# DecodeGenetics/graphtyper

Hardware: AMD Instinct MI355X
Metric: aligned+genotyped reads/sec over 1 Mb graph region; VCF bit-identical (higher is better)
Workload: dtype u64/u32 integer (2-bit k-mer keys, byte compares, u32 atomics)

## Files before the change

graphtyper_amd/csrc/gtx_api.hip:

```cpp
#include <hip/hip_runtime.h>
#include <chrono>

#include <algorithm>
#include <cstdio>
#include <cstdlib>
#include <cstring>
#include <memory>
#include <string>

#include "gtx_ctx.hpp"

#include <map>
#include "gtx_devmem.hpp"
#include "wave_hip.hpp"
#include "align_core.hpp"
#include "gtx_hbm_passes.hpp"
#include "score_core.hpp"
#include "score_replay.hpp"

namespace gtx
{
#ifdef GTX_PROF
constexpr uint64_t PROF_LOG_ENTRIES = 1u << 16, PROF_LOG_ENTRY = 16;
#else
// ... 1885 lines not shown
  CallScratch * const s = a.s;
  AlignRequest const & r = a.r;
  uint32_t const n = r.n_reads;
  uint32_t * const counters = s->d_counters;
  char const * fb = std::getenv("GTX_FORCE_SECOND_PASS");
  uint32_t const force = fb ? static_cast<uint32_t>(std::atoi(fb)) : 0u;
  uint32_t const n_cu = static_cast<uint32_t>(c->n_cu > 0 ? c->n_cu : 256);
  uint32_t const force_both = static_cast<uint32_t>(c->params.force_align_both_orientations != 0);
  char const * e4 = std::getenv("GTX_EXPRESS4");
  char const * eh = std::getenv("GTX_HINT");
  bool const four = !(e4 && e4[0] == '0');
  a.hinted = four && !(eh && eh[0] == '0');
  bool const wide = e4 && e4[0] == 'w' ? true : e4 && e4[0] == 'l' ? false : c->express4_wide;
  uint64_t const chunks = (static_cast<uint64_t>(n) + TASK_CHUNK - 1) / TASK_CHUNK;
  uint32_t const express4_per_cu = static_cast<uint32_t>(wide ? c->express4_wide_blocks_per_cu : c->express4_blocks_per_cu);
  a.mark(0, r.stream);
  if (a.hinted)
  {
    bool const sv_skips_express = c->params.is_sv_graph != 0 && force == 0;
    char const * hb = std::getenv("GTX_HINT_BUILD");
    bool const hint_dense = hb && hb[0] == 'd' ? true : hb && hb[0] == 'l' ? false : c->express4_wide;
    bool const hint_long = r.seq_stride > HintGeom<AlignCfg::KC>::ROW_BYTES;
    uint32_t const hint_threads = 64u * ((hint_long || hint_dense) ? GTX_HINT_WAVES : GTX_HINT_WAVES_LEAN);
    hipLaunchKernelGGL(hint_long ? gtx_align_hinted_long_kernel : hint_dense ? gtx_align_hinted_dense_kernel : gtx_align_hinted_kernel,
                       dim3((n + hint_threads - 1u) / hint_threads), dim3(hint_threads), 0, r.stream, c->dev_graph, c->dev_index, r.seq, r.seq_stride,
                       r.meta, n, r.records, r.rec_words, force_both, s->d_queue1.get(), s->d_queue.get(), reinterpret_cast<unsigned long long *>(counters + 2),
                       static_cast<uint32_t>(force != 0 || (eh && eh[0] == 'd')) | (sv_skips_express ? 4u : 0u)
#ifdef GTX_PROF
                         | (eh && eh[0] == 'x' ? 2u : 0u)
#endif
                         ,
                       r.task_flags, r.compact, a.timed && s->h_span.get() ? s->d_span : static_cast<unsigned long long *>(nullptr), a.var_masks);
    if (!hip_ok(hipGetLastError(), "gtx_align_hinted_kernel launch"))
      return GTX_ERR_HIP;
  }
  a.mark(1, r.stream);
  if (r.front_event)
  {
    (void)hipEventRecord(r.front_event, r.stream);
    if (r.tail_stream && r.tail_stream != r.stream)
    {
      (void)hipStreamWaitEvent(r.tail_stream, r.front_event, 0);
      a.sq = r.tail_stream;
    }
  }
  if (a.hinted)
  {
    uint32_t const blocks4q = static_cast<uint32_t>(std::min<uint64_t>((static_cast<uint64_t>(n) + 3u) / 4u, static_cast<uint64_t>(n_cu) * express4_per_cu));
// ... 1093 lines not shown
```

graphtyper_amd/csrc/gtx_flat.hpp:

```cpp
#pragma once
#include <algorithm>
#include <cstdlib>
#include <cstdint>
#include <string>
#include <vector>

#include "../../include/gtx.h"

namespace gtx
{
constexpr uint32_t K = GTX_K;
constexpr uint32_t INVALID = GTX_INVALID_ID;
constexpr uint32_t SPECIAL_START = GTX_SPECIAL_START;
constexpr uint32_t POS_BUCKET_SHIFT = 6;
constexpr uint32_t MAX_ALLELES = 32u * GTX_WIDE_MASK_WORDS;

struct alignas(8) uint2_t
{
  uint32_t x, y;
};

struct alignas(16) DevLabel
{
  uint32_t start, end;
// ... 55 lines not shown
};

constexpr uint32_t HINT_WIN_BEFORE = 160, HINT_WIN_ALLELE_MAX = 64, HINT_WIN_STRIDE = 384;
struct HintWindow
{
  uint32_t site, allele, len_a , len_0 ;
  uint32_t site_order , pad[3];
};

struct IndexView
{
  const IndexSlot * slots;
  const DevLabel * labels;
  uint32_t log2_cap;
  uint32_t max_index_labels;
  const IndexSlot * hslots;
  const HalfEntry * hlist;
  uint32_t h_log2_cap;
  uint32_t half_bucket_cap;
  const uint32_t * refp;
  const uint2_t * pos_flags;
  const uint2_t * tail_info;
  const uint32_t * filt[2];
  uint32_t hint_first, n_hint, filt_log2 , pad_hint;
  const HintWindow * win;
  const uint32_t * site_win;
  uint32_t win_base, n_win, pad_win[2];
};

#if defined(__HIPCC__)
__host__ __device__
#endif
inline uint32_t hint_win_base(uint32_t n_hint)
{
  return (n_hint / 64u + 5u) * 64u;
}
#if defined(__HIPCC__)
__host__ __device__
#endif
inline uint64_t hint_total_positions(uint32_t n_hint, uint32_t n_win)
{
  return n_win == 0 ? n_hint : static_cast<uint64_t>(hint_win_base(n_hint)) + static_cast<uint64_t>(n_win) * HINT_WIN_STRIDE + 256u;
}

constexpr uint32_t HINT_EXACT_OK = 1u, HINT_SINGLE_OK = 2u, HINT_L1 = 4u, HINT_R1 = 8u, HINT_PAR = 16u, HINT_ALT_OK = 32u;
constexpr uint32_t HINT_MULTI = 64u;
constexpr uint32_t HINT_TWO = 128u;
// ... 4 lines not shown
constexpr uint32_t HINT_SNP_GROUP = 1u << 21, HINT_REFB_SHIFT = 22u, HINT_NV_SHIFT = 24u;
constexpr uint32_t HINT_FAR_LEFT_SHIFT = 27u, HINT_FAR_RIGHT_SHIFT = 29u;
constexpr uint32_t HINT_NEAR_FREE = 1u << 31;
#if defined(__HIPCC__)
__host__ __device__
#endif
constexpr uint32_t hint_far_need(uint32_t m)
{
  return m <= 1 ? 1u : m == 2 ? 2u : m <= 6 ? 3u : 4u;
}
constexpr uint32_t HINT_TAIL_NODE = 2u;
constexpr uint32_t HINT_TAIL_OK = 1u, HINT_TAIL_NALL_SHIFT = 2u, HINT_TAIL_NEXT_SHIFT = 8u, HINT_TAIL_CODES_SHIFT = 16u;
constexpr uint32_t HINT_HE_CAP = 16, HINT_NB_MAX = 16;

inline uint32_t hint_filter_log2_words(uint64_t n_keys)
{
  uint32_t fl = 5;
  while ((1ull << fl) < n_keys + 1 && fl < 28)
    ++fl;
  uint32_t extra = 2;
  if (char const * e = std::getenv("GTX_FILTER_BITS_LOG2"))
    extra = static_cast<uint32_t>(std::max(5, std::min(9, std::atoi(e))) - 5);
  return std::min<uint32_t>(fl + extra, 28u);
}

#if defined(__HIPCC__)
__host__ __device__
#endif
inline void hint_filter_hash(uint32_t w0, uint32_t w1, uint32_t & h, uint32_t & h2)
{
  h = w1 * 0x9E3779B1u;
  h ^= h >> 15;
  h += w0;
  h *= 0x85EBCA77u;
  h ^= h >> 16;
  h2 = h * 0x9E3779B1u;
}
#if defined(__HIPCC__)
__host__ __device__
#endif
inline void hint_filter_slot_of(uint32_t h, uint32_t h2, uint32_t log2_words, uint32_t & word, uint32_t & mask)
{
  word = log2_words >= 32 ? h : h >> (32 - log2_words);
  mask = (1u << (h2 >> 27)) | (1u << ((h2 >> 22) & 31u)) | (1u << ((h2 >> 17) & 31u)) | (1u << ((h2 >> 12) & 31u));
}
#if defined(__HIPCC__)
// ... 138 lines not shown
```

graphtyper_amd/csrc/gtx_host.cpp:

```cpp
#include <algorithm>
#include <chrono>
#include <cstdio>
#include <cstdlib>
#include <cstring>
#include <numeric>
#include <thread>

#include "gtx_flat.hpp"
#include "index_build.hpp"

namespace gtx
{
GraphView HostGraph::view() const
{
  GraphView v{};
  v.n_ref = static_cast<uint32_t>(ref_order.size());
  v.n_var = static_cast<uint32_t>(var_order.size());
  v.n_special = static_cast<uint32_t>(special_actual.size());
  v.n_bucket = static_cast<uint32_t>(pos_bucket.size());
  v.first_order = ref_order.empty() ? 0 : ref_order[0];
  v.padding = padding;
  v.is_sv_graph = is_sv_graph;
  v.ref_order = ref_order.data();
  v.ref_len = ref_len.data();
// ... 522 lines not shown
    for (uint32_t i : l)
      bucket_insert(slots, log2_buckets, items[i]);
}

IndexView HostIndex::view(uint32_t max_index_labels, uint32_t half_bucket_cap) const
{
  IndexView ix{};
  ix.slots = slots.data();
  ix.labels = dev_labels.data();
  ix.log2_cap = log2_cap;
  ix.max_index_labels = max_index_labels;
  ix.hslots = hslots.data();
  ix.hlist = hlist.data();
  ix.h_log2_cap = h_log2_cap;
  ix.half_bucket_cap = half_bucket_cap;
  ix.refp = refp.data();
  ix.pos_flags = pos_flags.data();
  ix.tail_info = tail_info.data();
  ix.filt[0] = filt[0].data();
  ix.filt[1] = filt[1].data();
  ix.hint_first = hint_first;
  ix.n_hint = n_hint;
  ix.filt_log2 = filt_log2;
  ix.win = win.data();
  ix.site_win = site_win.data();
  ix.win_base = win_base;
  ix.n_win = static_cast<uint32_t>(win.size());
  return ix;
}

void hint_graph_tables(HostGraph const & g, HintGraphTables & t)
{
  uint32_t const R = static_cast<uint32_t>(g.ref_order.size());
  t = HintGraphTables();
  t.hint_first = g.ref_order.empty() ? 0 : g.ref_order[0] - 1;
  if (R == 0 || R - 1 >= HINT_NO_SITE)
    return;
  uint32_t const first = g.ref_order[0], last = g.ref_order[R - 1] + g.ref_len[R - 1];
  uint32_t const n = last - first;
  t.n = n;
  t.base.assign(n, 15);
  t.room.assign(n, 0);
  t.back.assign(n, 0);
  auto nib = [](char c) -> uint8_t { return c == 'A' ? 1 : c == 'C' ? 2 : c == 'G' ? 4 : c == 'T' ? 8 : 15; };
  for (uint32_t r = 0; r < R; ++r)
  {
// ... 515 lines not shown
```

graphtyper_amd/csrc/hinted.hpp:

```cpp
#pragma once
#include <type_traits>

#include "graph_dev.hpp"

namespace gtx
{
#ifdef GTX_EMU_NOTES
void hint_note(uint32_t code);
#define GTX_HINT_NOTE(code) hint_note(code)
#else
#define GTX_HINT_NOTE(code) ((void)0)
#endif

#ifdef GTX_X_STOP_AT
#define GTX_X_STOP(n, v)                                                                                                          \
  if (GTX_X_STOP_AT == (n))                                                                                                      \
  return static_cast<uint32_t>((v) == 0xA5A5A5A5u ? 2u : 0u)
#else
#define GTX_X_STOP(n, v) ((void)0)
#endif
constexpr uint32_t HINT_MAX_READ = 160;
constexpr uint32_t HINT_WORDS = HINT_MAX_READ / 8;

GTX_DEV uint32_t hint_bswap(uint32_t v)
// ... 249 lines not shown
  h.more |= prefix << 8;
}

enum : uint32_t
{
  HINT_K_DECLINE = 0,
  HINT_K_LABEL = 1,
  HINT_K_HOLE = 2
};

constexpr uint32_t HK_MM = 4u, HK_PAR = 8u, HK_ALLELE_SHIFT = 4u, HK_SET_SHIFT = 8u, HK_SITE_SHIFT = 16u;
constexpr uint32_t HK_TWO = 1u << HK_ALLELE_SHIFT;
GTX_DEV bool hk_is_two(uint32_t km)
{
  return (km & HK_TWO) != 0 && ((km >> HK_SET_SHIFT) & 255u) != 0;
}

GTX_DEV uint32_t hk_make(uint32_t kind, uint32_t site, uint32_t allele, bool mm, bool par)
{
  return kind | (mm ? HK_MM : 0u) | (par ? HK_PAR : 0u) | (allele << HK_ALLELE_SHIFT) | (site << HK_SITE_SHIFT);
}

constexpr uint32_t HK_NEED_LEFT = 64u, HK_NEED_RIGHT = 128u;

template <uint32_t I, bool DENSE, class Row, class Counts>
GTX_DEV uint32_t hint_kmer_judge(uint2_t const f, Row row, Counts const & h, uint32_t & amb2)
{
  constexpr uint32_t A = (K - 1) * I;
  uint32_t mis = hc_get(h.k[I], HC_MIS), mis_left = hc_get(h.k[I], HC_MIS_LEFT);
  uint32_t amb = hc_get(h.k[I], HC_AMB), amb_left = hc_get(h.k[I], HC_AMB_LEFT);
  uint32_t amb_out = hc_get(h.k[I], HC_AMB_OUT);
  uint32_t const site = f.x >> HINT_SITE_SHIFT;
  uint32_t const declined = hk_make(HINT_K_DECLINE, site, 0u, false, false);
  bool const several = DENSE && (f.x & (HINT_MULTI | HINT_TWO)) != 0 && (f.x & HINT_EXACT_OK) != 0;
  bool const single = (f.x & HINT_SINGLE_OK) != 0 || several;
  uint32_t const own_set = several ? (((f.x >> HINT_ALTIDX_SHIFT) & 255u) << HK_SET_SHIFT) | ((f.x & HINT_TWO) ? HK_TWO : 0u) : 0u;
  bool gl = single && (f.x & HINT_L1) != 0, gr = single && (f.x & HINT_R1) != 0;
  uint32_t const far_l = DENSE && single ? (f.y >> HINT_FAR_LEFT_SHIFT) & 3u : 0u, far_r = DENSE && single ? (f.y >> HINT_FAR_RIGHT_SHIFT) & 3u : 0u;
  auto GL = [&](uint32_t m) { return gl || far_l >= hint_far_need(m); };
  auto GR = [&](uint32_t m) { return gr || far_r >= hint_far_need(m); };
  if (amb == 0 && mis == 0)
  {
    if constexpr (DENSE)
      if ((f.x & HINT_TWO) != 0)
        return hk_make(HINT_K_LABEL, site, 0u, false, (f.x & HINT_PAR) != 0) | HK_TWO | (((f.x >> HINT_ALTIDX_SHIFT) & 255u) << HK_SET_SHIFT);
    bool const exact_ok = DENSE ? (f.x & HINT_EXACT_OK) != 0 : (f.x & (HINT_EXACT_OK | HINT_TWO)) == HINT_EXACT_OK;
// ... 29 lines not shown
      --amb;
      amb_left -= off < K / 2 ? 1u : 0u;
      amb_out -= ((rb >> refb) & 1u) ? 0u : 1u;
      site_set = (rb >> refb) & 1u;
#pragma unroll
      for (uint32_t b = 0; b < 4; ++b)
      {
        uint32_t const a = (f.x >> (HINT_ALTIDX_SHIFT + 2 * b)) & 3u;
        site_set |= (a != 0 && ((rb >> b) & 1u)) ? 1u << a : 0u;
      }
    }
    if (group)
    {
      gl = gr = true;
      site_left = off < K / 2;
    }
  }
  uint32_t const mis_right = mis - mis_left, amb_right = amb - amb_left;
  if (site_amb)
  {
    uint32_t const amb_far = site_left ? amb_right : amb_left, mis_far = site_left ? mis_right : mis_left;
    if (amb_far != 0 || amb > 1)
    {
      GTX_HINT_NOTE(7);
      return declined;
    }
    if (mis == 0)
      return hk_make((site_set != 0 && amb_out == 0) ? HINT_K_LABEL : HINT_K_HOLE, site, 0u, false, true) | (site_set << HK_SET_SHIFT);
    return hk_make(HINT_K_HOLE, site, 0u, false, true) | (mis_far == 0 ? 0u : site_left ? HK_NEED_RIGHT : HK_NEED_LEFT);
  }
  if (third)
  {
    uint32_t const need_site = site_left ? HK_NEED_LEFT : HK_NEED_RIGHT, need_far = site_left ? HK_NEED_RIGHT : HK_NEED_LEFT;
    uint32_t const amb_far = site_left ? amb_right : amb_left, mis_far = site_left ? mis_right : mis_left;
    if (amb == 0)
    {
      if (mis == 0)
        return hk_make(HINT_K_LABEL, site, 0u, true, false) | (((1u << ((f.y >> HINT_NV_SHIFT) & 7u)) - 1u) << HK_SET_SHIFT) | need_site;
      return hk_make(HINT_K_HOLE, site, 0u, false, false) | need_site | (mis_far != 0 ? need_far : 0u);
    }
    if (amb_far == 0 && mis_far == 0)
      return hk_make(HINT_K_HOLE, site, 0u, false, true);
    if (amb - amb_far == 0)
      return hk_make(HINT_K_HOLE, site, 0u, false, true) | need_site;
    GTX_HINT_NOTE(12);
    return declined;
  }
// ... 2 lines not shown
  if (amb == 2 && mis == 0 && (amb_left == 0 || amb_left == 2))
  {
    if (!(amb_left == 2 ? GR(1) : GL(1)))
    {
      GTX_HINT_NOTE(5);
      return declined;
    }
    return hk_make(amb_out == 0 ? HINT_K_LABEL : HINT_K_HOLE, site, allele, false, true) | own_set;
  }
  if (amb == 2 && mis == 0 && amb_left == 1 && GL(1))
  {
    amb2 |= 1u << I;
    return hk_make(amb_out == 0 ? HINT_K_LABEL : HINT_K_HOLE, site, allele, false, true) | own_set;
  }
  if (amb != 0 && mis != 0)
  {
    if (mis_left != 0 && amb_left == 0)
      return hk_make(HINT_K_HOLE, site, 0u, false, true) | HK_NEED_LEFT;
    if (mis_right != 0 && amb_right == 0)
      return hk_make(HINT_K_HOLE, site, 0u, false, true) | HK_NEED_RIGHT;
  }
  if (amb > 1)
  {
    GTX_HINT_NOTE(7);
    return declined;
  }
  if (amb == 0)
  {
    if (mis == 1)
    {
      bool const left = mis_left == 1;
      if (!(left ? GR(1) : GL(1)))
      {
        GTX_HINT_NOTE(3);
        return declined;
      }
      return hk_make(HINT_K_LABEL, site, allele, true, false) | (left ? HK_NEED_LEFT : HK_NEED_RIGHT) | own_set;
    }
    bool const ok = (mis_left != 0 || GL(mis)) && (mis_right != 0 || GR(mis));
    GTX_HINT_NOTE(ok ? 0 : 6);
    return hk_make(ok ? HINT_K_HOLE : HINT_K_DECLINE, site, 0u, false, false) | (mis_left != 0 ? HK_NEED_LEFT : 0u) |
           (mis_right != 0 ? HK_NEED_RIGHT : 0u);
  }
  bool const amb_is_left = amb_left == 1;
  if (mis == 0)
  {
    if (!(amb_is_left ? GR(1) : GL(1)))
    {
// ... 219 lines not shown
    return g.first_order + p;
  };
  uint32_t const n_k = 1 + (L - K) / (K - 1);
  HintCounts h{};
  uint32_t const * refw = ix.refp + 4 * (idx >> 5);
  uint32_t const sh = idx & 31u;
  uint2_t const f0 = ix.pos_flags[idx], f1 = ix.pos_flags[idx + (K - 1)];
  uint2_t const f2 = ix.pos_flags[idx + (n_k > 2 ? 2 * (K - 1) : 0u)], f3 = ix.pos_flags[idx + (n_k > 3 ? 3 * (K - 1) : 0u)];
  uint2_t const f4 = ix.pos_flags[idx + (n_k > 4 ? 4 * (K - 1) : 0u)];
  uint32_t const y_end = ix.pos_flags[idx + (K - 1) * n_k].y;
  uint2_t const t_end = ix.tail_info[idx + (K - 1) * n_k];
  GTX_X_STOP(0, f0.x ^ f1.y ^ f2.x ^ f3.y ^ f4.x ^ y_end ^ t_end.x ^ t_end.y ^ refw[0]);
  hint_compare(row, seq_stride, refw, sh, L, h);
  mm_all = hc_all(h);
  GTX_X_STOP(1, h.k[0] ^ h.k[1] ^ h.k[2] ^ h.k[3] ^ h.k[4] ^ h.upto ^ h.more ^ f0.x ^ f1.y ^ f2.x ^ f3.y ^ f4.x ^ y_end ^ t_end.x);
  uint32_t const none = hk_make(HINT_K_HOLE, HINT_NO_SITE, 0u, false, false);
  uint32_t amb2 = 0;
  uint32_t k0 = hint_kmer<0, DENSE>(f0, row, h, amb2), k1 = hint_kmer<1, DENSE>(f1, row, h, amb2);
  uint32_t k2 = n_k > 2 ? hint_kmer<2, DENSE>(f2, row, h, amb2) : none;
  uint32_t k3 = n_k > 3 ? hint_kmer<3, DENSE>(f3, row, h, amb2) : none;
  uint32_t k4 = n_k > 4 ? hint_kmer<4, DENSE>(f4, row, h, amb2) : none;
  if ((k0 & 3u) == HINT_K_DECLINE || (k1 & 3u) == HINT_K_DECLINE || (k2 & 3u) == HINT_K_DECLINE || (k3 & 3u) == HINT_K_DECLINE ||
      (k4 & 3u) == HINT_K_DECLINE)
    return false;
  GTX_X_STOP(2, k0 ^ (k1 << 1) ^ (k2 << 2) ^ (k3 << 3) ^ (k4 << 4) ^ amb2 ^ h.upto ^ h.more ^ y_end ^ t_end.x);
  if ((k0 | k1 | k2 | k3 | k4) & (HK_NEED_LEFT | HK_NEED_RIGHT))
  {
    uint32_t need = ((k0 >> 6) & 3u) | (((k1 >> 6) & 3u) << 2) | (((k2 >> 6) & 3u) << 4) | (((k3 >> 6) & 3u) << 6) | (((k4 >> 6) & 3u) << 8);
    static_assert(HK_NEED_LEFT == 64u && HK_NEED_RIGHT == 128u, "bit 2 I + side of `need`");
    bool maybe = false;
#ifndef GTX_X_NO_FILTER
    while (need != 0)
    {
      uint32_t const j0 = static_cast<uint32_t>(__builtin_ctz(need));
      need &= need - 1u;
      uint32_t a0, a1, word0, mask0, x1 = 0, mask1 = 1u;
      plane_extract16_at(row, (K - 1) * (j0 >> 1) + 16u * (j0 & 1u), a0, a1);
      hint_filter_slot(a0, a1, ix.filt_log2, word0, mask0);
      uint32_t const x0 = ix.filt[j0 & 1u][word0];
      if (need != 0)
      {
        uint32_t const j1 = static_cast<uint32_t>(__builtin_ctz(need));
        need &= need - 1u;
        uint32_t b0, b1, word1;
        plane_extract16_at(row, (K - 1) * (j1 >> 1) + 16u * (j1 & 1u), b0, b1);
        hint_filter_slot(b0, b1, ix.filt_log2, word1, mask1);
        x1 = ix.filt[j1 & 1u][word1];
      }
      maybe = maybe || (x0 & mask0) == mask0 || (x1 & mask1) == mask1;
    }
#endif
    if (maybe)
    {
      GTX_HINT_NOTE(4);
      return false;
    }
  }
  if ((k0 & 3u) == HINT_K_DECLINE || (k1 & 3u) == HINT_K_DECLINE || (k2 & 3u) == HINT_K_DECLINE || (k3 & 3u) == HINT_K_DECLINE ||
      (k4 & 3u) == HINT_K_DECLINE)
    return false;
  if (amb2 != 0)
  {
    if ((amb2 & (amb2 - 1u)) != 0)
    {
      GTX_HINT_NOTE(7);
      return false;
    }
    uint32_t const A = (K - 1) * static_cast<uint32_t>(__builtin_ctz(amb2));
    uint32_t p[4];
#pragma unroll
    for (uint32_t b = 0; b < 4; ++b)
    {
      uint32_t const w = A >> 5, sft = A & 31u;
      uint32_t const lo_w = row[4 * w + b], hi_w = row[4 * (w + 1 < HINT_PLANE_WORDS ? w + 1 : w) + b];
      p[b] = hint_funnel(lo_w, hi_w, sft) & 0xFFFFu;
    }
    uint32_t const odd = p[0] ^ p[1] ^ p[2] ^ p[3], three = (p[0] & p[1] & (p[2] | p[3])) | (p[2] & p[3] & (p[0] | p[1]));
    uint32_t const amb16 = ~(odd & ~three) & 0xFFFFu;
    uint32_t const j = static_cast<uint32_t>(__builtin_ctz(amb16 | 0x10000u)) & 15u;
    uint32_t const q = idx + A + j;
    uint32_t const * rq = ix.refp + 4 * (q >> 5);
    uint32_t const qs = q & 31u;
    uint32_t const rc = ((rq[0] >> qs) & 1u) | (((rq[1] >> qs) & 1u) << 1) | (((rq[2] >> qs) & 1u) << 2) | (((rq[3] >> qs) & 1u) << 3);
    uint32_t const ref_two = rc == 1 ? 0u : rc == 2 ? 1u : rc == 4 ? 2u : 3u;
    uint32_t const lo0 = (p[1] | p[3]) & ~(1u << j), hi0 = (p[2] | p[3]) & ~(1u << j);
    bool maybe = (rc & (rc - 1u)) != 0 || (amb16 & (amb16 - 1u)) != 0;
    uint32_t w3[3], m3[3];
#pragma unroll
// ... 18 lines not shown
           ((k4 & flag) == want ? 16u : 0u);
  };
  uint32_t const labelled = bits(3u, HINT_K_LABEL), par = bits(HK_PAR, HK_PAR), mmk = bits(HK_MM, HK_MM);
  uint32_t lo = 0, hi = n_k - 1;
  bool par_start = false;
  bool decided = false;
  uint32_t two_rs = 0, two_re = 0, two_mism = 0;
  if (labelled != (1u << n_k) - 1u)
  {
    uint32_t const x0 = labelled, x1 = x0 & (x0 >> 1), x2 = x1 & (x1 >> 1), x3 = x2 & (x2 >> 1), x4 = x3 & (x3 >> 1);
    static_assert(AlignCfg::KC == 5, "runs of up to five k-mers");
    uint32_t const deepest = x4 ? x4 : x3 ? x3 : x2 ? x2 : x1 ? x1 : x0;
    uint32_t const best_len = (x0 != 0 ? 1u : 0u) + (x1 != 0 ? 1u : 0u) + (x2 != 0 ? 1u : 0u) + (x3 != 0 ? 1u : 0u) + (x4 != 0 ? 1u : 0u);
    uint32_t const n_best = static_cast<uint32_t>(__builtin_popcount(deepest));
    uint32_t best_lo = deepest ? static_cast<uint32_t>(__builtin_ctz(deepest)) : 0u;
    uint32_t const second_lo = deepest ? 31u - static_cast<uint32_t>(__builtin_clz(deepest)) : 0u;
    uint32_t const second = (best_len == 0 || n_best >= 2) ? best_len : 0u;
    if (best_len <= second)
    {
      uint32_t const a_lo = best_lo, b_lo = second_lo, len = best_len;
      uint32_t const run_a = ((1u << len) - 1u) << a_lo, run_b = ((1u << len) - 1u) << b_lo;
      if (best_len == 0 || n_best != 2 || (f0.y & 255u) < L || (par & (run_a | run_b)) != 0)
      {
        GTX_HINT_NOTE(10);
        return HINT_TO_GENERAL;
      }
      uint32_t const all = hc_all(h);
      auto upto = [&](uint32_t j) { return j == 0 ? 0u : hc_upto(h, j); };
      auto cap = [](uint32_t n, uint32_t best) { return 2u + n / 11u < best ? 2u + n / 11u : best; };
      uint32_t best = 7;
      uint32_t const head_a = upto(a_lo) + (a_lo ? hc_edge(h, a_lo) : 0u), head_b = upto(b_lo) + hc_edge(h, b_lo);
      bool got_a = a_lo != 0 && head_a <= cap((K - 1) * a_lo + 1u, best);
      best = got_a ? head_a : best;
      bool const got_b = head_b <= cap((K - 1) * b_lo + 1u, best);
      got_a = got_a && !(got_b && head_b < best);
      uint32_t const rs_a = (got_a || a_lo == 0) ? 0u : (K - 1) * a_lo, rs_b = got_b ? 0u : (K - 1) * b_lo;
      uint32_t mm_a = static_cast<uint32_t>(__builtin_popcount(mmk & run_a)) + (got_a ? head_a : 0u);
      uint32_t mm_b = static_cast<uint32_t>(__builtin_popcount(mmk & run_b)) + (got_b ? head_b : 0u);
      uint32_t const end_a = (K - 1) * (a_lo + len), end_b = (K - 1) * (b_lo + len);
      uint32_t const tail_a = all - upto(a_lo + len), tail_b = all - upto(b_lo + len);
      best = 7;
      bool end_ok_a = tail_a <= cap(L - end_a, best);
      best = end_ok_a ? tail_a : best;
      bool const end_ok_b = end_b != L - 1 && tail_b <= cap(L - end_b, best);
      end_ok_a = end_ok_a && !(end_ok_b && tail_b < best);
      uint32_t const re_a = end_ok_a ? L - 1 : end_a, re_b = (end_ok_b || end_b == L - 1) ? L - 1 : end_b;
      mm_a += end_ok_a ? tail_a : 0u;
      mm_b += end_ok_b ? tail_b : 0u;
      uint32_t const size_a = re_a - rs_a + 1u, size_b = re_b - rs_b + 1u;
      if (size_a == size_b)
      {
        GTX_HINT_NOTE(10);
        return HINT_TO_GENERAL;
      }
      bool const a_wins = size_a > size_b;
      decided = true;
      two_rs = a_wins ? rs_a : rs_b;
      two_re = a_wins ? re_a : re_b;
      two_mism = a_wins ? mm_a : mm_b;
      best_lo = a_wins ? a_lo : b_lo;
    }
    par_start = !decided && best_lo > 0 && ((par >> best_lo) & 1u) != 0;
    lo = best_lo;
    hi = best_lo + best_len - 1;
  }
  uint32_t const run = ((2u << hi) - 1u) & ~((1u << lo) - 1u);
  uint32_t mism = static_cast<uint32_t>(__builtin_popcount(mmk & run));
  GTX_X_STOP(4, lo ^ (hi << 3) ^ (mism << 6) ^ (two_rs << 9) ^ (two_re << 17) ^ (two_mism << 25) ^ k0 ^ k1 ^ k2 ^ k3 ^ k4 ^ h.upto ^ h.more ^ y_end ^ t_end.x ^ static_cast<uint32_t>(decided) ^ static_cast<uint32_t>(par_start));
  uint32_t const prs = (K - 1) * lo, pre = (K - 1) * (hi + 1);
  uint32_t start = order_of(idx + prs), rs = prs;
  auto site_choice = [&](uint32_t tx, uint32_t rc0, uint32_t only, uint32_t & mask, uint32_t & x0) -> uint32_t
  {
    uint32_t const rc = rc0 == 0 ? 15u : rc0;
    uint32_t const nall = (tx >> HINT_TAIL_NALL_SHIFT) & 7u, codes = tx >> HINT_TAIL_CODES_SHIFT;
    uint32_t best = 2;
// ... 238 lines not shown
  push(4, k4);
  push(3, k3);
  push(2, k2);
  push(1, k1);
  push(0, k0);
  if (head_mask != 0)
    append((head_site << 16) | head_mask);
  if (clash || nvar > 6 || 6 + 3 * nvar > rec_words)
  {
    GTX_HINT_NOTE(13);
    return false;
  }
  uint32_t np = 1, longest = re - rs + 1;
  if (par_start && rs == 0)
  {
    uint32_t const amb_lo = hc_get(lo == 1 ? h.k[1] : lo == 2 ? h.k[2] : lo == 3 ? h.k[3] : h.k[4], HC_AMB);
    uint2_t const f_lo = lo == 1 ? f1 : lo == 2 ? f2 : lo == 3 ? f3 : f4;
    bool two_chains = amb_lo != 0;
    if (!two_chains)
    {
      uint32_t const off = (f_lo.y >> HINT_SNPOFF_SHIFT) & 31u;
      if ((f_lo.x & HINT_ALT_OK) == 0 || off == K - 1)
      {
        GTX_HINT_NOTE(10);
        return HINT_TO_GENERAL;
      }
      two_chains = off != 0;
    }
    if (two_chains)
    {
      uint32_t const mm_run = mmk & run, km_hi = hi == 0 ? k0 : hi == 1 ? k1 : hi == 2 ? k2 : hi == 3 ? k3 : k4;
      auto plain = [&](uint32_t k, uint32_t km) { return ((run >> k) & 1u) == 0 || (km & ((3u << HK_ALLELE_SHIFT) | (255u << HK_SET_SHIFT))) == 0; };
      if (!(plain(0, k0) && plain(1, k1) && plain(2, k2) && plain(3, k3) && plain(4, k4)))
      {
        GTX_HINT_NOTE(10);
        return HINT_TO_GENERAL;
      }
      bool const region_clean = hc_upto(h, hi + 1) == hc_upto(h, lo);
      if (mm_run == (1u << hi) && hi + 1 > 4)
      {
        GTX_HINT_NOTE(10);
        return HINT_TO_GENERAL;
      }
      bool const last_only = mm_run == (1u << hi) && hc_edge(h, hi + 1) == 1 && ((km_hi >> HK_SET_SHIFT) & 255u) == 0;
      bool const twin = region_clean && (mm_run == 0 || last_only);
      if (pre == L - 1 || re != L - 1 || (twin && nvar > 1))
      {
        GTX_HINT_NOTE(10);
        return HINT_TO_GENERAL;
      }
      if (twin && mm_run == 0)
        np = 2;
      else if (twin)
        --mism;
    }
  }
  if (mism > 10)
  {
    np = 0;
    longest = 0;
  }
  uint32_t const path_words = 4 + 3 * nvar;
  if (2 + np * path_words > rec_words)
    return false;
  bool const to_stage = stage != nullptr && rec_words >= HINT_STAGE_WORDS && 2 + (np ? np : 1u) * path_words <= HINT_STAGE_WORDS;
  uint32_t * rec = to_stage ? stage : hint_rec_ptr(rec_at);
  if (to_stage)
  {
#pragma unroll
    for (uint32_t k = 2; k < HINT_STAGE_WORDS; ++k)
      rec[k] = 0u;
// ... 90 lines not shown
```

graphtyper_amd/csrc/hinted_long.hpp:

```cpp
#pragma once
#include "hinted.hpp"

namespace gtx
{
template <uint32_t NK>
struct HintGeom
{
  static_assert(NK == 5 || NK == 8, "five k-mers (160 bases) or eight (256)");
  static constexpr uint32_t MAX_READ = NK == 5 ? 160u : 256u;
  static constexpr uint32_t PLANE_WORDS = MAX_READ / 32u;
  static constexpr uint32_t ROW_BYTES = MAX_READ / 2u;
};

template <uint32_t NK>
struct HintCountsN
{
  uint32_t k[NK];
  uint32_t upto, more, upto2;
};

template <uint32_t NK>
GTX_DEV uint32_t hc_upto(HintCountsN<NK> const & h, uint32_t j)
{
  if constexpr (NK == 5)
// ... 128 lines not shown
{
  constexpr uint32_t PW = HintGeom<NK>::PLANE_WORDS;
  uint32_t const L = m.l_qseq;
  auto order_of = [&](uint32_t p) -> uint32_t { return g.first_order + p; };
  uint32_t const n_k = 1 + (L - K) / (K - 1);
  HintCountsN<NK> h{};
  uint32_t const * refw = ix.refp + 4 * (idx >> 5);
  uint32_t const sh = idx & 31u;
  uint32_t fx[NK], fy[NK];
#pragma unroll
  for (uint32_t i = 0; i < NK; ++i)
  {
    uint2_t const f = ix.pos_flags[idx + ((i < 2 || i < n_k) ? i * (K - 1) : 0u)];
    fx[i] = f.x;
    fy[i] = f.y;
  }
  uint32_t const y_end = ix.pos_flags[idx + (K - 1) * n_k].y;
  uint2_t const t_end = ix.tail_info[idx + (K - 1) * n_k];
  hint_compare_n<NK>(row, seq_stride, refw, sh, L, h);
  uint32_t const none = hk_make(HINT_K_HOLE, HINT_NO_SITE, 0u, false, false);
  uint32_t amb2 = 0;
  uint32_t kv[NK];
  hint_kmers<0, NK>(kv, fx, fy, row, h, n_k, none, amb2);
  auto any_declined = [&]()
  {
    bool d = false;
#pragma unroll
    for (uint32_t i = 0; i < NK; ++i)
      d = d || (kv[i] & 3u) == HINT_K_DECLINE;
    return d;
  };
  if (any_declined())
    return false;
  uint32_t k_any = 0;
#pragma unroll
  for (uint32_t i = 0; i < NK; ++i)
    k_any |= kv[i];
  if (k_any & (HK_NEED_LEFT | HK_NEED_RIGHT))
  {
    uint32_t wl[NK], ml[NK], wr[NK], mr[NK], xl[NK], xr[NK];
    hint_probe_slots<0, NK>(ix, kv, row, wl, ml, wr, mr);
    uint32_t const * fl = ix.filt[0];
    uint32_t const * fr = ix.filt[1];
#pragma unroll
    for (uint32_t i = 0; i < NK; ++i)
    {
      xl[i] = fl[wl[i]];
      xr[i] = fr[wr[i]];
    }
#pragma unroll
    for (uint32_t i = 0; i < NK; ++i)
      kv[i] = hint_probe_verdict(kv[i], xl[i], ml[i], xr[i], mr[i]);
  }
  if (any_declined())
    return false;
  if (amb2 != 0)
  {
    if ((amb2 & (amb2 - 1u)) != 0)
    {
      GTX_HINT_NOTE(7);
      return false;
    }
    uint32_t const A = (K - 1) * static_cast<uint32_t>(__builtin_ctz(amb2));
    uint32_t p[4];
#pragma unroll
    for (uint32_t b = 0; b < 4; ++b)
    {
      uint32_t const w = A >> 5, sft = A & 31u;
      uint32_t const lo_w = row[4 * w + b], hi_w = row[4 * (w + 1 < PW ? w + 1 : w) + b];
      p[b] = hint_funnel(lo_w, hi_w, sft) & 0xFFFFu;
    }
    uint32_t const odd = p[0] ^ p[1] ^ p[2] ^ p[3], three = (p[0] & p[1] & (p[2] | p[3])) | (p[2] & p[3] & (p[0] | p[1]));
    uint32_t const amb16 = ~(odd & ~three) & 0xFFFFu;
    uint32_t const j = static_cast<uint32_t>(__builtin_ctz(amb16 | 0x10000u)) & 15u;
    uint32_t const q = idx + A + j;
    uint32_t const * rq = ix.refp + 4 * (q >> 5);
    uint32_t const qs = q & 31u;
    uint32_t const rc = ((rq[0] >> qs) & 1u) | (((rq[1] >> qs) & 1u) << 1) | (((rq[2] >> qs) & 1u) << 2) | (((rq[3] >> qs) & 1u) << 3);
    uint32_t const ref_two = rc == 1 ? 0u : rc == 2 ? 1u : rc == 4 ? 2u : 3u;
    uint32_t const lo0 = (p[1] | p[3]) & ~(1u << j), hi0 = (p[2] | p[3]) & ~(1u << j);
    bool maybe = (rc & (rc - 1u)) != 0 || (amb16 & (amb16 - 1u)) != 0;
    uint32_t w3[3], m3[3];
#pragma unroll
// ... 45 lines not shown
          best_lo = cur_lo;
          n_best = 1;
        }
        else if (cur_len != 0 && cur_len == best_len)
        {
          second = cur_len;
          second_lo = cur_lo;
          ++n_best;
        }
        else if (cur_len > second)
        {
          second = cur_len;
          second_lo = cur_lo;
        }
        cur_len = 0;
      }
    }
    if (best_len <= second)
    {
      uint32_t const a_lo = best_lo, b_lo = second_lo, len = best_len;
      uint32_t const run_a = ((1u << len) - 1u) << a_lo, run_b = ((1u << len) - 1u) << b_lo;
      if (best_len == 0 || n_best != 2 || (fy[0] & 255u) < L || (par & (run_a | run_b)) != 0)
      {
        GTX_HINT_NOTE(10);
        return HINT_TO_GENERAL;
      }
      uint32_t const all = hc_all(h);
      auto upto = [&](uint32_t j) { return j == 0 ? 0u : hc_upto(h, j); };
      auto cap = [](uint32_t n, uint32_t best) { return 2u + n / 11u < best ? 2u + n / 11u : best; };
      uint32_t best = 7;
      uint32_t const head_a = upto(a_lo) + (a_lo ? hc_edge(h, a_lo) : 0u), head_b = upto(b_lo) + hc_edge(h, b_lo);
      bool got_a = a_lo != 0 && head_a <= cap((K - 1) * a_lo + 1u, best);
      best = got_a ? head_a : best;
      bool const got_b = head_b <= cap((K - 1) * b_lo + 1u, best);
      got_a = got_a && !(got_b && head_b < best);
      uint32_t const rs_a = (got_a || a_lo == 0) ? 0u : (K - 1) * a_lo, rs_b = got_b ? 0u : (K - 1) * b_lo;
      uint32_t mm_a = static_cast<uint32_t>(__builtin_popcount(mmk & run_a)) + (got_a ? head_a : 0u);
      uint32_t mm_b = static_cast<uint32_t>(__builtin_popcount(mmk & run_b)) + (got_b ? head_b : 0u);
      uint32_t const end_a = (K - 1) * (a_lo + len), end_b = (K - 1) * (b_lo + len);
      uint32_t const tail_a = all - upto(a_lo + len), tail_b = all - upto(b_lo + len);
      best = 7;
      bool end_ok_a = tail_a <= cap(L - end_a, best);
      best = end_ok_a ? tail_a : best;
      bool const end_ok_b = end_b != L - 1 && tail_b <= cap(L - end_b, best);
      end_ok_a = end_ok_a && !(end_ok_b && tail_b < best);
      uint32_t const re_a = end_ok_a ? L - 1 : end_a, re_b = (end_ok_b || end_b == L - 1) ? L - 1 : end_b;
      mm_a += end_ok_a ? tail_a : 0u;
      mm_b += end_ok_b ? tail_b : 0u;
      uint32_t const size_a = re_a - rs_a + 1u, size_b = re_b - rs_b + 1u;
      if (size_a == size_b)
      {
        GTX_HINT_NOTE(10);
        return HINT_TO_GENERAL;
      }
      bool const a_wins = size_a > size_b;
      decided = true;
      two_rs = a_wins ? rs_a : rs_b;
      two_re = a_wins ? re_a : re_b;
      two_mism = a_wins ? mm_a : mm_b;
      best_lo = a_wins ? a_lo : b_lo;
    }
    par_start = !decided && best_lo > 0 && ((par >> best_lo) & 1u) != 0;
    lo = best_lo;
    hi = best_lo + best_len - 1;
  }
  uint32_t const run = ((2u << hi) - 1u) & ~((1u << lo) - 1u);
  uint32_t mism = static_cast<uint32_t>(__builtin_popcount(mmk & run));
  uint32_t const prs = (K - 1) * lo, pre = (K - 1) * (hi + 1);
  uint32_t start = order_of(idx + prs), rs = prs;
  auto site_choice = [&](uint32_t tx, uint32_t rc0, uint32_t only, uint32_t & mask, uint32_t & x0) -> uint32_t
  {
    uint32_t const rc = rc0 == 0 ? 15u : rc0;
    uint32_t const nall = (tx >> HINT_TAIL_NALL_SHIFT) & 7u, codes = tx >> HINT_TAIL_CODES_SHIFT;
    uint32_t best = 2;
    mask = 0;
// ... 162 lines not shown
  if (tail_mask != 0)
    append((tail_site << 16) | tail_mask);
#pragma unroll
  for (uint32_t j = 0; j < NK; ++j)
    push(NK - 1u - j, kv[NK - 1u - j]);
  if (head_mask != 0)
    append((head_site << 16) | head_mask);
  if (clash || nvar > 6 || 6 + 3 * nvar > rec_words)
  {
    GTX_HINT_NOTE(13);
    return false;
  }
  uint32_t np = 1, longest = re - rs + 1;
  if (par_start && rs == 0)
  {
    uint32_t const amb_lo = hc_get(hint_sel<1>(h.k, lo), HC_AMB);
    uint2_t const f_lo{hint_sel<1>(fx, lo), hint_sel<1>(fy, lo)};
    bool two_chains = amb_lo != 0;
    if (!two_chains)
    {
      uint32_t const off = (f_lo.y >> HINT_SNPOFF_SHIFT) & 31u;
      if ((f_lo.x & HINT_ALT_OK) == 0 || off == K - 1)
      {
        GTX_HINT_NOTE(10);
        return HINT_TO_GENERAL;
      }
      two_chains = off != 0;
    }
    if (two_chains)
    {
      uint32_t const mm_run = mmk & run, km_hi = hint_sel<0>(kv, hi);
      bool all_plain = true;
#pragma unroll
      for (uint32_t i = 0; i < NK; ++i)
        all_plain = all_plain && (((run >> i) & 1u) == 0 || (kv[i] & ((3u << HK_ALLELE_SHIFT) | (255u << HK_SET_SHIFT))) == 0);
      if (!all_plain)
      {
        GTX_HINT_NOTE(10);
        return HINT_TO_GENERAL;
      }
      bool const region_clean = hc_upto(h, hi + 1) == hc_upto(h, lo);
      if (mm_run == (1u << hi) && hi + 1 > NK - 1)
      {
        GTX_HINT_NOTE(10);
        return HINT_TO_GENERAL;
      }
      bool const last_only = mm_run == (1u << hi) && hc_edge(h, hi + 1) == 1 && ((km_hi >> HK_SET_SHIFT) & 255u) == 0;
      bool const twin = region_clean && (mm_run == 0 || last_only);
      if (pre == L - 1 || re != L - 1 || (twin && nvar > 1))
      {
        GTX_HINT_NOTE(10);
        return HINT_TO_GENERAL;
      }
      if (twin && mm_run == 0)
        np = 2;
      else if (twin)
        --mism;
    }
  }
  if (mism > 10)
  {
    np = 0;
    longest = 0;
  }
  uint32_t const path_words = 4 + 3 * nvar;
  if (2 + np * path_words > rec_words)
    return false;
  bool const to_stage = stage != nullptr && rec_words >= HINT_STAGE_WORDS && 2 + (np ? np : 1u) * path_words <= HINT_STAGE_WORDS;
  if (to_stage)
  {
    rec = stage;
#pragma unroll
    for (uint32_t k = 2; k < HINT_STAGE_WORDS; ++k)
      rec[k] = 0u;
// ... 52 lines not shown
```

Baseline: 17.78 billion.

## Resolve single ambiguous k-mer declines in hinted fast path instead of falling back

The hinted express aligner now records a compact summary of a k-mer it declined for ambiguity (2-3 candidates) and, when exactly one k-mer is declined and one side is resolvable, rewrites it as a label or hole instead of abandoning the fast path. The two-chain check also tolerates one non-plain k-mer by adjusting the region-clean comparison. Both are meant to keep more reads on the cheap hinted path and off the general aligner, at the cost of extra branches and a pos_flags load. A GTX_HINT_MORE=0 switch disables the extension, and the diagnostic note codes are split into finer categories.

```diff
diff --git a/graphtyper_amd/csrc/gtx_api.hip b/graphtyper_amd/csrc/gtx_api.hip
--- a/graphtyper_amd/csrc/gtx_api.hip
+++ b/graphtyper_amd/csrc/gtx_api.hip
@@ -1931,8 +1931,10 @@
     bool const hint_dense = hb && hb[0] == 'd' ? true : hb && hb[0] == 'l' ? false : c->express4_wide;
     bool const hint_long = r.seq_stride > HintGeom<AlignCfg::KC>::ROW_BYTES;
     uint32_t const hint_threads = 64u * ((hint_long || hint_dense) ? GTX_HINT_WAVES : GTX_HINT_WAVES_LEAN);
+    IndexView hint_index = c->dev_index;
+    hint_index.hint_less = hint_less_from_env();
     hipLaunchKernelGGL(hint_long ? gtx_align_hinted_long_kernel : hint_dense ? gtx_align_hinted_dense_kernel : gtx_align_hinted_kernel,
-                       dim3((n + hint_threads - 1u) / hint_threads), dim3(hint_threads), 0, r.stream, c->dev_graph, c->dev_index, r.seq, r.seq_stride,
+                       dim3((n + hint_threads - 1u) / hint_threads), dim3(hint_threads), 0, r.stream, c->dev_graph, hint_index, r.seq, r.seq_stride,
                        r.meta, n, r.records, r.rec_words, force_both, s->d_queue1.get(), s->d_queue.get(), reinterpret_cast<unsigned long long *>(counters + 2),
                        static_cast<uint32_t>(force != 0 || (eh && eh[0] == 'd')) | (sv_skips_express ? 4u : 0u)
 #ifdef GTX_PROF
diff --git a/graphtyper_amd/csrc/gtx_flat.hpp b/graphtyper_amd/csrc/gtx_flat.hpp
--- a/graphtyper_amd/csrc/gtx_flat.hpp
+++ b/graphtyper_amd/csrc/gtx_flat.hpp
@@ -101,7 +101,7 @@
   const uint2_t * pos_flags;
   const uint2_t * tail_info;
   const uint32_t * filt[2];
-  uint32_t hint_first, n_hint, filt_log2 , pad_hint;
+  uint32_t hint_first, n_hint, filt_log2 , hint_less;
   const HintWindow * win;
   const uint32_t * site_win;
   uint32_t win_base, n_win, pad_win[2];
@@ -152,6 +152,12 @@
   if (char const * e = std::getenv("GTX_FILTER_BITS_LOG2"))
     extra = static_cast<uint32_t>(std::max(5, std::min(9, std::atoi(e))) - 5);
   return std::min<uint32_t>(fl + extra, 28u);
+}
+
+inline uint32_t hint_less_from_env()
+{
+  char const * e = std::getenv("GTX_HINT_MORE");
+  return e && e[0] == '0' ? 1u : 0u;
 }
 
 #if defined(__HIPCC__)
diff --git a/graphtyper_amd/csrc/gtx_host.cpp b/graphtyper_amd/csrc/gtx_host.cpp
--- a/graphtyper_amd/csrc/gtx_host.cpp
+++ b/graphtyper_amd/csrc/gtx_host.cpp
@@ -568,6 +568,7 @@
   ix.hint_first = hint_first;
   ix.n_hint = n_hint;
   ix.filt_log2 = filt_log2;
+  ix.hint_less = hint_less_from_env();
   ix.win = win.data();
   ix.site_win = site_win.data();
   ix.win_base = win_base;
diff --git a/graphtyper_amd/csrc/hinted.hpp b/graphtyper_amd/csrc/hinted.hpp
--- a/graphtyper_amd/csrc/hinted.hpp
+++ b/graphtyper_amd/csrc/hinted.hpp
@@ -295,6 +295,9 @@
 }
 
 constexpr uint32_t HK_NEED_LEFT = 64u, HK_NEED_RIGHT = 128u;
+constexpr uint32_t HS_SHIFT = 8u, HS_VALID = 1u, HS_KMER_SHIFT = 1u, HS_GL = 1u << 4, HS_GR = 1u << 5, HS_NEAR = 1u << 6, HS_SNP_HALF_SHIFT = 7u,
+                   HS_SUBST_LEFT = 1u << 9, HS_SUBST_RIGHT = 1u << 10, HS_AMB_LEFT_SHIFT = 11u, HS_AMB_RIGHT_SHIFT = 13u,
+                   HS_SET_MISSES = 1u << 15, HS_ALLELE_SHIFT = 16u, HS_MANY = 1u << 18;
 
 template <uint32_t I, bool DENSE, class Row, class Counts>
 GTX_DEV uint32_t hint_kmer_judge(uint2_t const f, Row row, Counts const & h, uint32_t & amb2)
@@ -370,7 +373,7 @@
     uint32_t const amb_far = site_left ? amb_right : amb_left, mis_far = site_left ? mis_right : mis_left;
     if (amb_far != 0 || amb > 1)
     {
-      GTX_HINT_NOTE(7);
+      GTX_HINT_NOTE(71);
       return declined;
     }
     if (mis == 0)
@@ -419,8 +422,19 @@
   }
   if (amb > 1)
   {
-    GTX_HINT_NOTE(7);
-    return declined;
+    GTX_HINT_NOTE(72);
+    if constexpr (std::is_same<Counts, HintCounts>::value)
+      if (amb <= 3u)
+      {
+        uint32_t const off = (f.x & HINT_ALT_OK) != 0 ? (f.y >> HINT_SNPOFF_SHIFT) & 31u : 32u;
+        auto one = [](uint32_t n) { return n < 1u ? n : 1u; };
+        uint32_t const w = HS_VALID | (I << HS_KMER_SHIFT) | (GL(mis + amb) ? HS_GL : 0u) | (GR(mis + amb) ? HS_GR : 0u) |
+                           ((f.y >> 31) * HS_NEAR) | ((off >> 4) << HS_SNP_HALF_SHIFT) | (one(mis_left) * HS_SUBST_LEFT) | (one(mis_right) * HS_SUBST_RIGHT) |
+                           (amb_left << HS_AMB_LEFT_SHIFT) | (amb_right << HS_AMB_RIGHT_SHIFT) | (one(amb_out) * HS_SET_MISSES) | (allele << HS_ALLELE_SHIFT);
+        static_assert(HINT_NEAR_FREE == 1u << 31, "bit 31 of the second flag word");
+        amb2 |= ((amb2 >> HS_SHIFT) != 0 ? HS_MANY : w) << HS_SHIFT;
+      }
+    return declined | own_set;
   }
   if (amb == 0)
   {
@@ -686,7 +700,35 @@
   uint32_t k4 = n_k > 4 ? hint_kmer<4, DENSE>(f4, row, h, amb2) : none;
   if ((k0 & 3u) == HINT_K_DECLINE || (k1 & 3u) == HINT_K_DECLINE || (k2 & 3u) == HINT_K_DECLINE || (k3 & 3u) == HINT_K_DECLINE ||
       (k4 & 3u) == HINT_K_DECLINE)
-    return false;
+  {
+    uint32_t const sv = amb2 >> HS_SHIFT;
+    if (sv == 0 || (sv & HS_MANY) != 0 || ix.hint_less != 0)
+      return false;
+    uint32_t const n_declined = ((k0 & 3u) == HINT_K_DECLINE ? 1u : 0u) + ((k1 & 3u) == HINT_K_DECLINE ? 1u : 0u) + ((k2 & 3u) == HINT_K_DECLINE ? 1u : 0u) +
+                                ((k3 & 3u) == HINT_K_DECLINE ? 1u : 0u) + ((k4 & 3u) == HINT_K_DECLINE ? 1u : 0u);
+    uint32_t const amb_l = (sv >> HS_AMB_LEFT_SHIFT) & 3u, amb_r = (sv >> HS_AMB_RIGHT_SHIFT) & 3u;
+    bool const near = (sv & HS_NEAR) != 0;
+    uint32_t const snp_half = (sv >> HS_SNP_HALF_SHIFT) & 3u;
+    bool const left_known = (sv & HS_SUBST_LEFT) == 0 && (sv & HS_GL) != 0 && (amb_l == 0 || (amb_l == 1 && near && snp_half != 0));
+    bool const right_known = (sv & HS_SUBST_RIGHT) == 0 && (sv & HS_GR) != 0 && (amb_r == 0 || (amb_r == 1 && near && snp_half != 1));
+    if (n_declined != 1 || !(left_known || right_known))
+    {
+      GTX_HINT_NOTE(72);
+      return false;
+    }
+    uint32_t const i = (sv >> HS_KMER_SHIFT) & 7u;
+    uint32_t const km = i == 0 ? k0 : i == 1 ? k1 : i == 2 ? k2 : i == 3 ? k3 : k4;
+    bool const no_subst = (sv & (HS_SUBST_LEFT | HS_SUBST_RIGHT)) == 0;
+    uint32_t const v = no_subst ? hk_make((sv & HS_SET_MISSES) == 0 ? HINT_K_LABEL : HINT_K_HOLE, km >> HK_SITE_SHIFT, (sv >> HS_ALLELE_SHIFT) & 3u, false, true) |
+                                    (km & ((255u << HK_SET_SHIFT) | HK_TWO))
+                                : hk_make(HINT_K_HOLE, km >> HK_SITE_SHIFT, 0u, false, true);
+    k0 = i == 0 ? v : k0;
+    k1 = i == 1 ? v : k1;
+    k2 = i == 2 ? v : k2;
+    k3 = i == 3 ? v : k3;
+    k4 = i == 4 ? v : k4;
+  }
+  amb2 &= (1u << HS_SHIFT) - 1u;
   GTX_X_STOP(2, k0 ^ (k1 << 1) ^ (k2 << 2) ^ (k3 << 3) ^ (k4 << 4) ^ amb2 ^ h.upto ^ h.more ^ y_end ^ t_end.x);
   if ((k0 | k1 | k2 | k3 | k4) & (HK_NEED_LEFT | HK_NEED_RIGHT))
   {
@@ -727,7 +769,7 @@
   {
     if ((amb2 & (amb2 - 1u)) != 0)
     {
-      GTX_HINT_NOTE(7);
+      GTX_HINT_NOTE(73);
       return false;
     }
     uint32_t const A = (K - 1) * static_cast<uint32_t>(__builtin_ctz(amb2));
@@ -792,7 +834,7 @@
       uint32_t const run_a = ((1u << len) - 1u) << a_lo, run_b = ((1u << len) - 1u) << b_lo;
       if (best_len == 0 || n_best != 2 || (f0.y & 255u) < L || (par & (run_a | run_b)) != 0)
       {
-        GTX_HINT_NOTE(10);
+        GTX_HINT_NOTE(best_len == 0 ? 101 : n_best != 2 ? 102 : (f0.y & 255u) < L ? 103 : 104);
         return HINT_TO_GENERAL;
       }
       uint32_t const all = hc_all(h);
@@ -820,7 +862,7 @@
       uint32_t const size_a = re_a - rs_a + 1u, size_b = re_b - rs_b + 1u;
       if (size_a == size_b)
       {
-        GTX_HINT_NOTE(10);
+        GTX_HINT_NOTE(105);
         return HINT_TO_GENERAL;
       }
       bool const a_wins = size_a > size_b;
@@ -1105,7 +1147,7 @@
       uint32_t const off = (f_lo.y >> HINT_SNPOFF_SHIFT) & 31u;
       if ((f_lo.x & HINT_ALT_OK) == 0 || off == K - 1)
       {
-        GTX_HINT_NOTE(10);
+        GTX_HINT_NOTE(106);
         return HINT_TO_GENERAL;
       }
       two_chains = off != 0;
@@ -1114,22 +1156,33 @@
     {
       uint32_t const mm_run = mmk & run, km_hi = hi == 0 ? k0 : hi == 1 ? k1 : hi == 2 ? k2 : hi == 3 ? k3 : k4;
       auto plain = [&](uint32_t k, uint32_t km) { return ((run >> k) & 1u) == 0 || (km & ((3u << HK_ALLELE_SHIFT) | (255u << HK_SET_SHIFT))) == 0; };
-      if (!(plain(0, k0) && plain(1, k1) && plain(2, k2) && plain(3, k3) && plain(4, k4)))
-      {
-        GTX_HINT_NOTE(10);
-        return HINT_TO_GENERAL;
-      }
-      bool const region_clean = hc_upto(h, hi + 1) == hc_upto(h, lo);
+      uint32_t alt_sites = 0;
+      uint32_t const other = (plain(0, k0) ? 0u : 1u) | (plain(1, k1) ? 0u : 2u) | (plain(2, k2) ? 0u : 4u) | (plain(3, k3) ? 0u : 8u) | (plain(4, k4) ? 0u : 16u);
+      if (other != 0)
+      {
+        uint32_t const k = static_cast<uint32_t>(__builtin_ctz(other));
+        uint32_t const km = k == 0 ? k0 : k == 1 ? k1 : k == 2 ? k2 : k == 3 ? k3 : k4;
+        uint32_t const yk = ix.pos_flags[idx + (K - 1) * k].y;
+        bool ok = ix.hint_less == 0 && mm_run == 0 && pw == nullptr;
+        ok = ok && (other & (other - 1u)) == 0 && ((km >> HK_SET_SHIFT) & 255u) == 0;
+        alt_sites = (K - 1) * k + ((yk >> HINT_SNPOFF_SHIFT) & 31u) < pre ? 1u : 0u;
+        if (!ok)
+        {
+          GTX_HINT_NOTE(107);
+          return HINT_TO_GENERAL;
+        }
+      }
+      bool const region_clean = hc_upto(h, hi + 1) == hc_upto(h, lo) + alt_sites;
       if (mm_run == (1u << hi) && hi + 1 > 4)
       {
-        GTX_HINT_NOTE(10);
+        GTX_HINT_NOTE(108);
         return HINT_TO_GENERAL;
       }
       bool const last_only = mm_run == (1u << hi) && hc_edge(h, hi + 1) == 1 && ((km_hi >> HK_SET_SHIFT) & 255u) == 0;
       bool const twin = region_clean && (mm_run == 0 || last_only);
       if (pre == L - 1 || re != L - 1 || (twin && nvar > 1))
       {
-        GTX_HINT_NOTE(10);
+        GTX_HINT_NOTE(109);
         return HINT_TO_GENERAL;
       }
       if (twin && mm_run == 0)
diff --git a/graphtyper_amd/csrc/hinted_long.hpp b/graphtyper_amd/csrc/hinted_long.hpp
--- a/graphtyper_amd/csrc/hinted_long.hpp
+++ b/graphtyper_amd/csrc/hinted_long.hpp
@@ -174,6 +174,7 @@
   uint32_t amb2 = 0;
   uint32_t kv[NK];
   hint_kmers<0, NK>(kv, fx, fy, row, h, n_k, none, amb2);
+  amb2 &= (1u << HS_SHIFT) - 1u;
   auto any_declined = [&]()
   {
     bool d = false;
@@ -210,7 +211,7 @@
   {
     if ((amb2 & (amb2 - 1u)) != 0)
     {
-      GTX_HINT_NOTE(7);
+      GTX_HINT_NOTE(73);
       return false;
     }
     uint32_t const A = (K - 1) * static_cast<uint32_t>(__builtin_ctz(amb2));
@@ -302,7 +303,7 @@
       uint32_t const run_a = ((1u << len) - 1u) << a_lo, run_b = ((1u << len) - 1u) << b_lo;
       if (best_len == 0 || n_best != 2 || (fy[0] & 255u) < L || (par & (run_a | run_b)) != 0)
       {
-        GTX_HINT_NOTE(10);
+        GTX_HINT_NOTE(best_len == 0 ? 101 : n_best != 2 ? 102 : (fy[0] & 255u) < L ? 103 : 104);
         return HINT_TO_GENERAL;
       }
       uint32_t const all = hc_all(h);
@@ -330,7 +331,7 @@
       uint32_t const size_a = re_a - rs_a + 1u, size_b = re_b - rs_b + 1u;
       if (size_a == size_b)
       {
-        GTX_HINT_NOTE(10);
+        GTX_HINT_NOTE(105);
         return HINT_TO_GENERAL;
       }
       bool const a_wins = size_a > size_b;
@@ -539,7 +540,7 @@
       uint32_t const off = (f_lo.y >> HINT_SNPOFF_SHIFT) & 31u;
       if ((f_lo.x & HINT_ALT_OK) == 0 || off == K - 1)
       {
-        GTX_HINT_NOTE(10);
+        GTX_HINT_NOTE(106);
         return HINT_TO_GENERAL;
       }
       two_chains = off != 0;
@@ -553,20 +554,20 @@
         all_plain = all_plain && (((run >> i) & 1u) == 0 || (kv[i] & ((3u << HK_ALLELE_SHIFT) | (255u << HK_SET_SHIFT))) == 0);
       if (!all_plain)
       {
-        GTX_HINT_NOTE(10);
+        GTX_HINT_NOTE(107);
         return HINT_TO_GENERAL;
       }
       bool const region_clean = hc_upto(h, hi + 1) == hc_upto(h, lo);
       if (mm_run == (1u << hi) && hi + 1 > NK - 1)
       {
-        GTX_HINT_NOTE(10);
+        GTX_HINT_NOTE(108);
         return HINT_TO_GENERAL;
       }
       bool const last_only = mm_run == (1u << hi) && hc_edge(h, hi + 1) == 1 && ((km_hi >> HK_SET_SHIFT) & 255u) == 0;
       bool const twin = region_clean && (mm_run == 0 || last_only);
       if (pre == L - 1 || re != L - 1 || (twin && nvar > 1))
       {
-        GTX_HINT_NOTE(10);
+        GTX_HINT_NOTE(109);
         return HINT_TO_GENERAL;
       }
       if (twin && mm_run == 0)
```

Result: faster. 18.86 billion, median of 6 (+6.1%).
